# alibaba/nann

Hardware: AMD Instinct MI355X
Metric: retrieval QPS @ recall@200 parity, 1M items/128-d (higher is better)
Workload: dtype f16 rows / f32 L2

## Files before the change

### nann_amd/csrc/nann_hip.hip

```cpp
#include "nann_eval.h"
#include "nann_attn.h"
#include "nann_order_kernels.h"
#include "nann_scan.h"
#include "host/nann_graphdef_text.h"
#include "host/nann_blaze_options.h"
#include "host/nann_npy.h"
#include "host/nann_projcache.h"

#include <algorithm>
#include <atomic>
#include <cmath>
#include <cstddef>
#include <cstdio>
#include <cstdlib>
#include <cstring>
#include <fstream>
#include <limits>
#include <memory>
#include <mutex>
#include <string>
#include <vector>

#include <sys/stat.h>

// ... 548 lines not shown
  const int count = s_count;
  const uint16_t* h = reinterpret_cast<const uint16_t*>(seq_smem);
  for (int k = tid; k < d; k += kSeqMeanThreads) {
    float acc = 0.0f;
    for (int r = 0; r < seq_len; ++r) acc = acc + half_bits_to_float(h[r * d + k]);
    q[(long long)blockIdx.x * d + k] = count ? acc / (float)count : 0.0f;
  }
}

template <int LPR, int DT>
__global__ __launch_bounds__(256) void k_score_l2(const void* table, long long n_table_rows, int d,
                                                  const int32_t* indices, long long n,
                                                  const float* qv, float* scores, OpResult* res) {
  constexpr int GPW = 64 / LPR;
  const int lane = lane_id();
  const int sub = lane % LPR, grp = lane / LPR;
  float q[8];
#pragma unroll
  for (int k = 0; k < 8; ++k) q[k] = qv[sub * 8 + k];
  const long long wave_global = (long long)blockIdx.x * (blockDim.x >> 6) + wave_id();
  const long long n_waves = (long long)gridDim.x * (blockDim.x >> 6);
  for (long long i0 = wave_global * GPW; i0 < n; i0 += n_waves * GPW) {
    const long long i = i0 + grp;
    long long row = -1;
    if (i < n) {
      row = indices ? (long long)indices[i] : i;
      if (row < 0 || row >= n_table_rows) {
        if (sub == 0) atomicMin(reinterpret_cast<unsigned long long*>(&res->bad_i), (unsigned long long)i);
        row = -1;
      }
    }
    float x[8];
    if (row >= 0) {
      const RowChunk<DT> ch = load_chunk<DT>(table, (size_t)row, d, sub);
      chunk_to_float<DT>(ch, x);
    } else {
#pragma unroll
      for (int k = 0; k < 8; ++k) x[k] = 0.0f;
    }
    const float s = l2_finish<LPR>(q, x);
    if (sub == 0 && i < n) scores[i] = s;
  }
}

struct HipProjBackend {
  typedef hipStream_t Stream;
  typedef hipEvent_t Event;
  static bool malloc(void** p, size_t bytes) {
    if (hipMalloc(p, bytes) == hipSuccess) return true;
    (void)hipGetLastError();
    return false;
  }
  static void free(void* p) { (void)hipFree(p); }
  static bool mem_info(size_t* free_b) {
    size_t total = 0;
    if (hipMemGetInfo(free_b, &total) == hipSuccess) return true;
    (void)hipGetLastError();
    return false;
  }
  static bool event_create(Event* e) {
    if (hipEventCreateWithFlags(e, hipEventDisableTiming) == hipSuccess) return true;
    (void)hipGetLastError();
    return false;
  }
  static void event_destroy(Event e) { (void)hipEventDestroy(e); }
  static void event_record(Event e, Stream s) { (void)hipEventRecord(e, s); }
  static bool event_done(Event e) { return hipEventQuery(e) != hipErrorNotReady; }
  static void event_wait(Event e) { (void)hipEventSynchronize(e); }
};
typedef nann::ProjCacheT<HipProjBackend> ProjCache;
typedef nann::ProjTableT<HipProjBackend> ProjTable;
struct SearchOpt {
  int mode;
  int reserve;
  int preproject;
  int mlp_form;
  int small32;
  int order;
};
static std::atomic<int> g_traversal_mode{-1}, g_slot_reserve{-1}, g_preproject{-1};
static const SearchOpt& env_defaults() {
  static const SearchOpt d = [] {
    SearchOpt o{NANN_TRAVERSAL_AUTO, 0, 1, NANN_MLP_FORM_AUTO, 1, 1};
    if (const char* e = std::getenv("NANN_PREPROJECT")) o.preproject = !(e[0] == '0' && e[1] == 0);
    if (const char* e = std::getenv("NANN_SEARCH_SLOT_RESERVE")) o.reserve = std::max(0, std::atoi(e));
    if (const char* e = std::getenv("NANN_MLP_FORM")) o.mlp_form = std::string(e) == "fused" ? NANN_MLP_FORM_FUSED : std::string(e) == "phased" ? NANN_MLP_FORM_PHASED : NANN_MLP_FORM_AUTO;
    if (const char* e = std::getenv("NANN_PHASE_SMALL32")) o.small32 = !(e[0] == '0');
    if (const char* e = std::getenv("NANN_QUERY_ORDER")) o.order = !(e[0] == '0');
    return o;
  }();
  return d;
}
static SearchOpt resolve_options(const nann_search_options* u) {
  SearchOpt o = env_defaults();
  const int gm = g_traversal_mode.load(std::memory_order_relaxed), gr = g_slot_reserve.load(std::memory_order_relaxed),
            gp = g_preproject.load(std::memory_order_relaxed);
  if (gm >= 0) o.mode = gm;
  if (gr >= 0) o.reserve = gr;
  if (gp >= 0) o.preproject = gp;
  if (u) {
    const size_t nb = u->struct_bytes > 0 ? (size_t)u->struct_bytes : sizeof(*u);
    auto has = [&](const int32_t* f) { return (size_t)(reinterpret_cast<const char*>(f) - reinterpret_cast<const char*>(u)) + 4 <= nb; };
    if (has(&u->traversal_mode) && u->traversal_mode >= 0) o.mode = u->traversal_mode;
    if (has(&u->slot_reserve) && u->slot_reserve >= 0) o.reserve = u->slot_reserve;
    if (has(&u->preprojection) && u->preprojection >= 0) o.preproject = u->preprojection != 0;
    if (has(&u->mlp_form) && u->mlp_form >= 0) o.mlp_form = u->mlp_form;
  }
  return o;
}
static int check_options(const nann_search_options* u) {
  if (!u) return NANN_OK;
  if (u->struct_bytes < 0 || (u->struct_bytes > 0 && u->struct_bytes < 8)) return fail(NANN_ERR_BAD_ARGUMENT, "nann_search_options: struct_bytes");
  const SearchOpt o = resolve_options(u);
  if (o.mode < NANN_TRAVERSAL_AUTO || o.mode > NANN_TRAVERSAL_LDS_HASH32) return fail(NANN_ERR_BAD_ARGUMENT, "nann_search_options: unknown traversal_mode");
  if (o.mlp_form < NANN_MLP_FORM_AUTO || o.mlp_form > NANN_MLP_FORM_PHASED) return fail(NANN_ERR_BAD_ARGUMENT, "nann_search_options: unknown mlp_form");
  return NANN_OK;
}

struct nann_scorer {
  nann_scorer_desc desc;
  float* dev_weights = nullptr;
  uint4* dev_packed = nullptr;
  float4* dev_packed_x = nullptr;
  float* dev_cert = nullptr;
  MlpParams mlp = {};
  mutable ProjCache proj;
};

struct nann_attn_scorer {
  AttnParams P = {};
  int emb_dtype = 0;
  int precision = NANN_MLP_EXACT_F32;
  float* dev_weights = nullptr;
  uint4* dev_packed = nullptr;
  mutable ProjCache proj;
};

struct nann_index {
  nann_index_desc desc;
  uint64_t uid = 0;
  bool owns = false;
  std::vector<void*> owned;
  int64_t max_deg[2] = {0, 0};
  uint32_t bm_words = 0;
  bool probe_valid = false;
  int probe_ef = 0, probe_queries = 0;
  float probe_new_per_row_mean = 0.0f, probe_new_per_row_q90 = 0.0f, probe_new_per_row_max = 0.0f;
  float* pivots = nullptr;
  int n_pivots = 0;
};
static void probe_index(nann_index* ix);
static void choose_pivots(nann_index* ix, const std::vector<int32_t>& enter);
static int launch_order(const nann_index* ix, const float* q, int n, int32_t* key, int32_t* perm, unsigned int* heads,
                        hipStream_t st);

extern "C" {

int nann_abi_version(void) { return NANN_ABI_VERSION; }
const char* nann_last_error(void) { return nann::g_err.c_str(); }

int nann_device_count(void) {
  int n = 0;
  if (hipGetDeviceCount(&n) != hipSuccess) return 0;
  return n;
}

int nann_malloc(void** dev_ptr, int64_t nbytes) {
  if (!dev_ptr || nbytes < 0) return fail(NANN_ERR_BAD_ARGUMENT, "nann_malloc: bad argument");
  HIP_TRY(hipMalloc(dev_ptr, (size_t)std::max<int64_t>(nbytes, 1)));
  return NANN_OK;
}

int nann_free(void* dev_ptr) {
  if (dev_ptr) HIP_TRY(hipFree(dev_ptr));
  return NANN_OK;
}

int nann_memcpy(void* dst, const void* src, int64_t nbytes, int kind, nann_stream_t stream) {
  static const hipMemcpyKind kinds[3] = {hipMemcpyHostToDevice, hipMemcpyDeviceToHost,
                                         hipMemcpyDeviceToDevice};
  if (kind < 0 || kind > 2 || nbytes < 0) return fail(NANN_ERR_BAD_ARGUMENT, "nann_memcpy: bad argument");
  if (nbytes == 0) return NANN_OK;
  HIP_TRY(hipMemcpyAsync(dst, src, (size_t)nbytes, kinds[kind], as_stream(stream)));
  return NANN_OK;
}

int nann_stream_synchronize(nann_stream_t stream) {
  HIP_TRY(hipStreamSynchronize(as_stream(stream)));
  return NANN_OK;
}

int nann_stream_create(nann_stream_t* out) {
  if (!out) return fail(NANN_ERR_BAD_ARGUMENT, "nann_stream_create: null argument");
  hipStream_t s = nullptr;
  HIP_TRY(hipStreamCreateWithFlags(&s, hipStreamNonBlocking));
  *out = reinterpret_cast<nann_stream_t>(s);
  return NANN_OK;
}

int nann_stream_destroy(nann_stream_t stream) {
  if (!stream) return NANN_OK;
  HIP_TRY(hipStreamDestroy(as_stream(stream)));
  return NANN_OK;
}

int nann_host_malloc(void** host_ptr, int64_t nbytes) {
  if (!host_ptr || nbytes < 0) return fail(NANN_ERR_BAD_ARGUMENT, "nann_host_malloc: bad argument");
  HIP_TRY(hipHostMalloc(host_ptr, (size_t)std::max<int64_t>(nbytes, 1), hipHostMallocDefault));
  return NANN_OK;
}

int nann_host_free(void* host_ptr) {
  if (!host_ptr) return NANN_OK;
  HIP_TRY(hipHostFree(host_ptr));
  return NANN_OK;
}

static uint16_t f32_to_f16_rne(float f) { return nann_npy::f32_to_f16_rne(f); }

static int read_whole_file(const char* path, std::vector<unsigned char>* out) {
  std::ifstream f(path, std::ifstream::binary | std::ifstream::ate);
  if (!f) return fail(NANN_ERR_IO, std::string("Fail to open file: ") + path);
  const std::streamoff size = f.tellg();
  if (size < 0) return fail(NANN_ERR_IO, std::string("Fail to open file: ") + path);
  out->resize((size_t)size);
  f.seekg(0);
  if (size > 0) f.read(reinterpret_cast<char*>(out->data()), size);
  if (!f || f.gcount() != size) return fail(NANN_ERR_IO, std::string("short read of ") + path);
  return NANN_OK;
}

static int read_npy_host(const char* path, int expect_dtype, const int64_t* expect_shape, int expect_rank,
                         int allow_cast, std::vector<char>* out, std::vector<int64_t>* out_shape) {
  std::vector<unsigned char> image;
  int rc = read_whole_file(path, &image);
  if (rc) return rc;
  const unsigned char* payload = nullptr;
  size_t bytes = 0;
  std::vector<char> conv;
  std::string err;
  rc = nann_npy::decode(image.data(), image.size(), expect_dtype, expect_shape, expect_rank, allow_cast != 0, &payload, &bytes, &conv,
                        out_shape, &err);
  if (rc) return fail(rc, err);
  if (!conv.empty() || bytes == 0) { conv.resize(bytes); out->swap(conv); }
  else out->assign(reinterpret_cast<const char*>(payload), reinterpret_cast<const char*>(payload) + bytes);
  return NANN_OK;
}

int nann_huge_const_load(const char* path, int expect_dtype, const int64_t* expect_shape,
                         int expect_rank, int allow_cast, void** dev_ptr, int64_t* nbytes) {
  if (!path || !dev_ptr) return fail(NANN_ERR_BAD_ARGUMENT, "nann_huge_const_load: null argument");
  std::vector<unsigned char> image;
  int rc = read_whole_file(path, &image);
  if (rc) return rc;
  const unsigned char* payload = nullptr;
  size_t bytes = 0;
  std::vector<char> conv;
  std::string err;
  rc = nann_npy::decode(image.data(), image.size(), expect_dtype, expect_shape, expect_rank, allow_cast != 0, &payload, &bytes, &conv,
                        nullptr, &err);
  if (rc) return fail(rc, err);
  const int64_t total = (int64_t)bytes;
  void* d = nullptr;
  HIP_TRY(hipMalloc(&d, (size_t)std::max<int64_t>(total, 1)));
  if (total) {
    const hipError_t e = hipMemcpy(d, payload, (size_t)total, hipMemcpyHostToDevice);
    if (e != hipSuccess) {
      (void)hipFree(d);
      return fail(NANN_ERR_HIP, std::string("hipMemcpy: ") + hipGetErrorString(e));
    }
  }
  *dev_ptr = d;
  if (nbytes) *nbytes = total;
  return NANN_OK;
}

int nann_group_gather_count(const int64_t* params_row_splits, int64_t n_params_splits,
                            int64_t n_params_values, const int64_t* indices_values,
                            int64_t n_indices_values, const int64_t* indices_row_splits,
                            int64_t n_indices_splits, int64_t* ret_row_splits,
                            int64_t* scratch_offsets, int64_t* n_ret, int64_t* n_ret_splits,
                            int32_t* ragged_code, nann_stream_t stream) {
  if (!n_ret || !n_ret_splits) return fail(NANN_ERR_BAD_ARGUMENT, "nann_group_gather_count: null out");
  ResultBuf* rb;
  int rc = get_result_buf(&rb);
  if (rc) return rc;
  hipStream_t st = as_stream(stream);
  hipLaunchKernelGGL(k_group_gather_count, dim3(1), dim3(kNT), 0, st, params_row_splits,
                     (long long)n_params_splits, (long long)n_params_values, indices_values,
                     (long long)n_indices_values, indices_row_splits, (long long)n_indices_splits,
                     ret_row_splits, scratch_offsets, rb->dev);
  HIP_TRY(hipGetLastError());
  rc = fetch_result(rb, st);
  if (rc) return rc;
  if (ragged_code) *ragged_code = rb->host->code;
  *n_ret = rb->host->n_out;
  *n_ret_splits = rb->host->n_out_splits;
  if (rb->host->err) return fail(rb->host->err, "GroupGather: invalid input, code " +
                                                    std::to_string(rb->host->code));
  return NANN_OK;
}

int nann_group_gather_fill(const int32_t* params_values, const int64_t* params_row_splits,
                           const int64_t* indices_values, int64_t n_indices_values,
                           const int64_t* scratch_offsets, int32_t* ret_values,
                           nann_stream_t stream) {
  if (n_indices_values <= 0) return NANN_OK;
// ... 1115 lines not shown
  o->struct_bytes = (int32_t)sizeof(*o);
  o->traversal_mode = o->slot_reserve = o->preprojection = o->mlp_form = -1;
}

int nann_set_traversal_mode(int32_t mode) {
  if (mode < NANN_TRAVERSAL_AUTO || mode > NANN_TRAVERSAL_LDS_HASH32)
    return fail(NANN_ERR_BAD_ARGUMENT, "nann_set_traversal_mode: unknown mode");
  g_traversal_mode.store(mode, std::memory_order_relaxed);
  return NANN_OK;
}

int nann_search_workspace_bytes(const nann_index* ix, const int32_t level_topn[6], int64_t n_queries,
                                int64_t* nbytes) {
  if (!ix || !level_topn || !nbytes) return fail(NANN_ERR_BAD_ARGUMENT, "nann_search_workspace_bytes: null argument");
  SearchPlan p;
  const int rc = plan_search(ix, level_topn, n_queries, -1, &p, resolve_options(nullptr));
  if (rc) return rc;
  *nbytes = (int64_t)(256 + p.slot_bytes * (unsigned long long)std::max(p.slots, p.fb_slots) + kPhaseTail +
                      order_ws_bytes(n_queries));
  return NANN_OK;
}

}


template <typename Build>
static int projection_for(ProjCache& c, const nann_index* ix, int width, hipStream_t st, Build build, bool pin, bool enabled,
                          std::shared_ptr<ProjTable>* out) {
  const size_t bytes = (size_t)ix->desc.n_items * (size_t)width * 4;
  return c.acquire(ix->uid, bytes, enabled, pin, [&](float* t) -> int {
    const int rc = build(t);
    if (rc) return rc;
    const hipError_t e = hipStreamSynchronize(st);
    if (e != hipSuccess) return fail(NANN_ERR_HIP, std::string("pre-projection: ") + hipGetErrorString(e));
    return NANN_OK;
  }, out);
}

static void projection_used(ProjCache& c, const std::shared_ptr<ProjTable>& tab, hipStream_t st) { c.used(tab, st); }

static int projection_release(ProjCache& c, const nann_index* ix) {
  if (c.release(ix->uid)) return NANN_OK;
  return fail(NANN_ERR_BAD_ARGUMENT, "release: no pre-projected table of this index");
}

static int mlp_projection(const nann_scorer* sc, const nann_index* ix, hipStream_t st, bool pin, bool enabled, std::shared_ptr<ProjTable>* out) {
  return projection_for(sc->proj, ix, kMlpProjWidth, st, [&](float* t) {
    return launch_mlp_preproject(ix->desc.emb_dtype, ix->desc.item_embs, (long long)ix->desc.n_items, ix->desc.d, sc->mlp.w1, t, st);
  }, pin, enabled, out);
}

static int attn_projection(const nann_attn_scorer* sc, const nann_index* ix, hipStream_t st, bool pin, bool enabled, std::shared_ptr<ProjTable>* out) {
  return projection_for(sc->proj, ix, kAttnProjWidth, st, [&](float* t) {
    return launch_attn_preproject(ix->desc.emb_dtype, sc->P, ix->desc.item_embs, (long long)ix->desc.n_items, t, st);
  }, pin, enabled, out);
}

static int launch_search_any(int lpr, int dt, int kind, int split, int vis, int nt, int slots, size_t lds_bytes,
                             const SearchArgs& a, hipStream_t st) {
  if (kind == NANN_SCORER_MLP) {
    if (lpr == 8) return launch_search_mlp_d64(dt, split, vis, slots, lds_bytes, a, st);
    if (lpr == 16) return launch_search_mlp_d128(dt, split, vis, slots, lds_bytes, a, st);
    if (lpr == 32) return launch_search_mlp_d256(dt, split, vis, slots, lds_bytes, a, st);
    return fail(NANN_ERR_UNSUPPORTED, "MLP scorer: d <= 256 only");
  }
  if (dt == NANN_F16) return launch_search_l2_f16(lpr, vis, nt, slots, lds_bytes, a, st);
  if (dt == NANN_BF16) return launch_search_l2_bf16(lpr, vis, nt, slots, lds_bytes, a, st);
  return launch_search_l2_f32(lpr, vis, nt, slots, lds_bytes, a, st);
}

extern "C" {

int nann_search(const nann_index* ix, const nann_scorer* scorer, const float* q, int64_t n_queries,
                const int32_t level_topn[6], void* workspace, int64_t workspace_bytes,
                int64_t* out_item_ids, float* out_scores, int32_t* out_index, int32_t* status,
                int32_t* counters, nann_stream_t stream) {
  return nann_search_opt(ix, scorer, q, n_queries, level_topn, nullptr, workspace, workspace_bytes, out_item_ids, out_scores,
                         out_index, status, counters, nullptr, nullptr, nullptr, stream);
}

}

static int search_impl(const nann_index* ix, const nann_scorer* scorer, const nann_attn_scorer* attn,
                       const float* q, const float* kt, const float* upad, int64_t n_queries,
                       const int32_t level_topn[6], const int32_t* tq, void* workspace, int64_t workspace_bytes,
                       int64_t* out_item_ids, float* out_scores, int32_t* out_index, int32_t* status,
                       int32_t* counters, int64_t* phase_ticks, const nann_search_options* options, nann_search_plan* plan_out,
                       hipStream_t st) {
  if (n_queries > 0x7fffffffll) return fail(NANN_ERR_UNSUPPORTED, "too many queries in one call");
  int rc = check_options(options);
  if (rc) return rc;
  SearchOpt opt = resolve_options(options);
  const int kind = attn ? kKindAttn : scorer->desc.kind;
  const bool mlp = !attn && kind == NANN_SCORER_MLP;
  const bool mlp_split = mlp && scorer->desc.precision == NANN_MLP_SPLIT_F16;
  const bool mlp_cert = mlp && scorer->desc.precision == NANN_MLP_CERTIFIED;
  if (mlp_cert && opt.mlp_form == NANN_MLP_FORM_FUSED) opt.mlp_form = NANN_MLP_FORM_PHASED;
  std::shared_ptr<ProjTable> tab;
  ProjCache* cache = nullptr;
  if (attn) {
    cache = &attn->proj;
    rc = attn_projection(attn, ix, st, false, opt.preproject != 0, &tab);
  } else if (mlp) {
    cache = &scorer->proj;
    rc = mlp_projection(scorer, ix, st, false, opt.preproject != 0, &tab);
  }
  if (rc) return rc;
  const bool mlp_res = mlp && tab;
  SearchPlan p;
  rc = plan_search(ix, level_topn, n_queries, mlp_res ? kKindMlpRes : mlp_split ? kKindMlpSplit : kind, &p, opt, mlp && !mlp_split);
  if (rc) return rc;
  if (plan_out) {
    const bool ph = mlp_res && p.phased;
    const int v = ph ? p.phase_vis : p.vis;
    plan_out->visited_set = v == VIS_LDS_HASH ? NANN_TRAVERSAL_LDS_HASH : v == VIS_LDS_HASH32 ? NANN_TRAVERSAL_LDS_HASH32
                            : v == VIS_LDS_BITMAP ? NANN_TRAVERSAL_LDS_BITMAP : NANN_TRAVERSAL_HBM_BITMAP;
    plan_out->fallback_visited_set = p.fb_vis == VIS_LDS_BITMAP ? NANN_TRAVERSAL_LDS_BITMAP : NANN_TRAVERSAL_HBM_BITMAP;
    plan_out->threads = ph ? (p.phase_vis == VIS_LDS_HASH32 ? kNT : 512) : ((mlp || attn) && p.nt == kNT ? 512 : p.nt);
    plan_out->workgroups = ph ? p.phase_slots : p.slots;
    plan_out->phased = ph ? 1 : 0;
    plan_out->table = tab ? 1 : 0;
    plan_out->est_visited = p.est_visited;
    plan_out->worst_visited = p.worst_visited;
  }
  const int64_t need_slots = p.phased ? std::max<int64_t>(std::min<int64_t>(n_queries, kPhaseChunk), p.fb_slots) : std::max(p.slots, p.fb_slots);
  if (!workspace || workspace_bytes < (int64_t)(256 + p.slot_bytes * (unsigned long long)need_slots + (p.phased ? kPhaseTail : 0)))
    return fail(NANN_ERR_CAPACITY, "workspace smaller than nann_search_workspace_bytes()");
  SearchArgs a;
  a.emb = ix->desc.item_embs;
  a.item_ids = ix->desc.item_ids;
  for (int l = 0; l < 2; ++l) { a.nbv[l] = ix->desc.nb_values[l]; a.nbrs[l] = ix->desc.nb_row_splits[l]; }
  a.enter = ix->desc.enter_points;
  a.n_enter = (int)ix->desc.n_enter;
  a.n_items = (uint32_t)ix->desc.n_items;
  a.d = ix->desc.d;
  a.q = q;
  a.n_queries = (int)n_queries;
  for (int i = 0; i < 6; ++i) a.t[i] = level_topn[i];
  a.tq = tq;
  a.ws = static_cast<unsigned char*>(workspace);
  a.slot_bytes = p.slot_bytes;
  a.bm_words = ix->bm_words;
  a.max_cand = p.max_cand; a.max_raw = p.max_raw; a.pool_cap = p.pool_cap;
  a.out_ids = out_item_ids; a.out_scores = out_scores; a.out_index = out_index;
  a.status = status; a.counters = counters;
  a.phase_ticks = reinterpret_cast<long long*>(phase_ticks);
  a.id_bits = p.id_bits;
  a.redo = 0;
  a.phase = 0;
  a.proj = tab ? tab->table : nullptr;
  a.mlp = MlpParams{};
  a.attn = AttnParams{};
  a.kt = kt; a.upad = upad;
  HIP_TRY(hipMemsetAsync(workspace, 0, 256, st));
  const int dt = ix->desc.emb_dtype;
  const bool hashed = p.vis == VIS_LDS_HASH || p.vis == VIS_LDS_HASH32;
  const unsigned long long slots_end = 256 + p.slot_bytes * (unsigned long long)std::max(p.slots, p.fb_slots) + kPhaseTail;
  const unsigned long long order_off = ((unsigned long long)workspace_bytes - order_ws_bytes(n_queries)) & ~255ull;
  if (opt.order && hashed && !attn && kind == NANN_SCORER_L2 && ix->n_pivots >= 2 && n_queries > p.slots &&
      (unsigned long long)workspace_bytes >= ((slots_end + 255) & ~255ull) + order_ws_bytes(n_queries)) {
    unsigned char* ow = static_cast<unsigned char*>(workspace) + order_off;
    unsigned int* heads = reinterpret_cast<unsigned int*>(ow);
    int32_t* perm = reinterpret_cast<int32_t*>(ow + kOrderSegs * kOrderHeadStride * 4);
    int32_t* key = perm + n_queries;
    rc = launch_order(ix, q, (int)n_queries, key, perm, heads, st);
    if (rc) return rc;
    a.perm = perm;
    a.xheads = heads;
  }
  auto both = [&](auto&& launch_on) -> int {
    int r2 = launch_on(p.vis, p.nt, p.slots, p.lds_bytes);
    if (!r2 && hashed) {
      a.redo = 1;
      a.perm = nullptr;
      a.xheads = nullptr;
      r2 = launch_on(p.fb_vis, kNT, p.fb_slots, p.fb_lds_bytes);
    }
    if (cache) projection_used(*cache, tab, st);
    return r2;
  };
  if (attn) {
    a.attn = attn->P;
    if (tab) {
      auto launch = attn->precision == NANN_MLP_SPLIT_F16 ? launch_search_attn_proj : launch_search_attn_xproj;
      const bool resident = attn->precision == NANN_MLP_SPLIT_F16;
      return both([&](int vis, int, int slots, size_t lds) {
        if (resident && vis == VIS_LDS_HASH && !a.redo) return launch_search_attn_res(slots, lds, a, st);
        return launch(vis, slots, lds, a, st);
      });
    }
    auto launch = attn->precision == NANN_MLP_SPLIT_F16 ? launch_search_attn_split : launch_search_attn;
    return both([&](int vis, int, int slots, size_t lds) { return launch(ix->desc.d, dt, vis, slots, lds, a, st); });
  }
  a.mlp = scorer->mlp;
  a.phase = 0;
  const int exact = scorer->desc.kind == NANN_SCORER_MLP && (scorer->desc.precision == NANN_MLP_EXACT_F32 || mlp_cert);
  if (mlp_res && p.phased) {
    DeviceInfo di;
    rc = device_info(&di);
    if (rc) return rc;
    const int k5 = level_topn[5];
    for (int64_t c0 = 0; c0 < n_queries && !rc; c0 += kPhaseChunk) {
      SearchArgs c = a;
      c.n_queries = (int)std::min<int64_t>(kPhaseChunk, n_queries - c0);
      c.q = q + (size_t)c0 * a.d;
      if (tq) c.tq = tq + (size_t)c0 * 6;
      c.out_ids = out_item_ids + (size_t)c0 * k5;
      if (out_scores) c.out_scores = out_scores + (size_t)c0 * k5;
      if (out_index) c.out_index = out_index + (size_t)c0 * k5;
      c.status = status + c0;
      if (counters) c.counters = counters + (size_t)c0 * 3 * NANN_NUM_ROUNDS;
      if (phase_ticks) c.phase_ticks = reinterpret_cast<long long*>(phase_ticks) + (size_t)c0 * NANN_NUM_PHASES;
      if (c0 && mlp_cert) {
        HIP_TRY(hipMemsetAsync(workspace, 0, offsetof(WsHeader, refined), st));
        HIP_TRY(hipMemsetAsync(static_cast<unsigned char*>(workspace) + offsetof(WsHeader, pad2), 0, 256 - offsetof(WsHeader, pad2), st));
      } else if (c0) HIP_TRY(hipMemsetAsync(workspace, 0, 256, st));
      const int slots = (int)std::min<int64_t>(c.n_queries, (int64_t)p.phase_slots);
      for (int ph = 0; ph <= NANN_NUM_ROUNDS && !rc; ++ph) {
        c.phase = ph;
        rc = launch_search_mlp_phase(p.phase_vis, slots, p.phase_lds_bytes, c, st);
        if (!rc && ph < NANN_NUM_ROUNDS) {
          rc = mlp_cert ? launch_mlp_phase_certified(c, ph, p.phase_score_wgs, st)
                        : launch_mlp_phase_score(exact, c, ph, p.phase_score_wgs, st);
        }
      }
      if (!rc) {
        c.redo = 1;
        c.phase = 0;
        rc = launch_search_mlp_res(exact, p.fb_vis, p.fb_slots, p.fb_lds_bytes, c, st);
      }
    }
    if (cache) projection_used(*cache, tab, st);
    return rc;
  }
  if (mlp_res)
    return both([&](int vis, int, int slots, size_t lds) {
      return launch_search_mlp_res(exact, vis, slots, lds, a, st);
    });
  return both([&](int vis, int nt, int slots, size_t lds) {
    return launch_search_any(ix->desc.d / 8, dt, kind, mlp_split, vis, nt, slots, lds, a, st);
  });
}

__global__ void k_probe_queries(const void* emb, int dt, int d, long long n_items, int nq, float* q) {
  const int j = blockIdx.x;
  const long long row = (long long)j * (n_items / nq);
  for (int k = threadIdx.x; k < d; k += blockDim.x) {
    float v;
    if (dt == NANN_F32) v = static_cast<const float*>(emb)[row * d + k];
    else {
      const uint32_t h = static_cast<const uint16_t*>(emb)[row * d + k];
      v = dt == NANN_F16 ? half_bits_to_float(h) : bf16_bits_to_float(h);
    }
    q[(size_t)j * d + k] = v;
  }
}

__global__ void k_order_gather(const void* emb, int dt, int d, const int32_t* rows, int m, float* out) {
  for (int k = threadIdx.x; k < d; k += blockDim.x) out[(size_t)blockIdx.x * d + k] = order_row_elem(emb, dt, (size_t)rows[blockIdx.x] * d + k);
}

static int launch_order(const nann_index* ix, const float* q, int n, int32_t* key, int32_t* perm, unsigned int* heads,
                        hipStream_t st) {
  const int d = ix->desc.d, P = ix->n_pivots;
  const size_t lds = ((size_t)d * P + kOrderMaxPivots + (size_t)kOrderKeyQueries * d) * 4;
  if (lds > 48 * 1024)
    HIP_TRY(hipFuncSetAttribute(reinterpret_cast<const void*>(k_order_key), hipFuncAttributeMaxDynamicSharedMemorySize, (int)lds));
  hipLaunchKernelGGL(k_order_key, dim3((unsigned)((n + kOrderKeyQueries - 1) / kOrderKeyQueries)), dim3(256), lds, st,
                     ix->pivots, d, P, q, n, key);
  HIP_TRY(hipGetLastError());
  hipLaunchKernelGGL(k_order_perm, dim3(1), dim3(kOrderSortThreads), 0, st, key, n, P, perm, heads);
  HIP_TRY(hipGetLastError());
  return NANN_OK;
}

static void choose_pivots(nann_index* ix, const std::vector<int32_t>& enter) {
  const int d = ix->desc.d;
  const int P = order_pivots((int64_t)enter.size(), d);
  if (P < 2) return;
  constexpr size_t kMaxCand = 1024;
  const size_t E = enter.size(), m = std::min(E, kMaxCand);
  std::vector<int32_t> cand(m);
  for (size_t i = 0; i < m; ++i) cand[i] = enter[i * E / m];
  int32_t* rows = nullptr;
  float* buf = nullptr;
  std::vector<float> x(m * (size_t)d);
  bool ok = hipMalloc(&rows, m * 4) == hipSuccess && hipMalloc(&buf, m * (size_t)d * 4) == hipSuccess &&
            hipMemcpy(rows, cand.data(), m * 4, hipMemcpyHostToDevice) == hipSuccess;
  if (ok) {
    hipLaunchKernelGGL(k_order_gather, dim3((unsigned)m), dim3(128), 0, nullptr, ix->desc.item_embs, ix->desc.emb_dtype, d, rows, (int)m, buf);
    ok = hipGetLastError() == hipSuccess && hipMemcpy(x.data(), buf, x.size() * 4, hipMemcpyDeviceToHost) == hipSuccess;
  }
  if (buf) (void)hipFree(buf);
  if (rows) (void)hipFree(rows);
  if (!ok) return;
  std::vector<size_t> piv;
  std::vector<double> dist(m, INFINITY);
  size_t cur = 0;
  for (int p = 0; p < P; ++p) {
    piv.push_back(cur);
    size_t far = cur;
    for (size_t i = 0; i < m; ++i) {
      double s = 0.0;
      for (int k = 0; k < d; ++k) { const double t = (double)x[i * d + k] - (double)x[cur * d + k]; s += t * t; }
      dist[i] = std::min(dist[i], s);
      if (dist[i] > dist[far]) far = i;
    }
    if (dist[far] <= 0.0) break;
    cur = far;
  }
  if (piv.size() < 2) return;
  const size_t np = piv.size();
  std::vector<float> t((size_t)d * np + kOrderMaxPivots, 0.0f);
  for (size_t p = 0; p < np; ++p) {
    float s = 0.0f;
    for (int k = 0; k < d; ++k) {
      const float v = x[piv[p] * d + k];
      t[(size_t)k * np + p] = v;
      s += v * v;
    }
    t[(size_t)d * np + p] = s;
  }
  float* dev = nullptr;
  if (hipMalloc(&dev, t.size() * 4) != hipSuccess) return;
  if (hipMemcpy(dev, t.data(), t.size() * 4, hipMemcpyHostToDevice) != hipSuccess) { (void)hipFree(dev); return; }
  ix->pivots = dev;
  ix->n_pivots = (int)piv.size();
}

static void probe_index(nann_index* ix) {
  ix->probe_valid = false;
  static const bool enabled = [] { const char* e = std::getenv("NANN_INDEX_PROBE"); return !(e && e[0] == '0'); }();
  if (!enabled) return;
  const std::string saved_error = nann::g_err;
  struct RestoreError { const std::string& s; ~RestoreError() { nann::g_err = s; } } restore{saved_error};
  const int d = ix->desc.d;
  const int64_t E = ix->desc.n_enter, N = ix->desc.n_items;
  if (E < 8 || N < 4096) return;
  const int nq = 64, e = (int)std::min<int64_t>(64, E);
  const int32_t t[6] = {e, e, e, e, e, std::min(e, 10)};
  nann_scorer_desc sd{};
  sd.kind = NANN_SCORER_L2; sd.d = d; sd.emb_dtype = ix->desc.emb_dtype;
  nann_scorer* sc = nullptr;
  if (nann_scorer_create(&sd, &sc) != NANN_OK) return;
  nann_search_options o;
  nann_search_options_init(&o);
  o.traversal_mode = NANN_TRAVERSAL_HBM_BITMAP;
  o.slot_reserve = 0;
  int64_t ws_bytes = 0;
  const size_t n_ctr = (size_t)nq * 3 * NANN_NUM_ROUNDS;
  unsigned char* buf = nullptr;
  std::vector<int32_t> h_ctr(n_ctr), h_st((size_t)nq);
  bool ok = nann_search_workspace_bytes(ix, t, nq, &ws_bytes) == NANN_OK;
  const size_t off_q = ((size_t)ws_bytes + 255) & ~(size_t)255, off_ids = off_q + (size_t)nq * d * 4,
               off_st = off_ids + (size_t)nq * t[5] * 8, off_ctr = off_st + (size_t)nq * 4, total = off_ctr + n_ctr * 4;
  ok = ok && hipMalloc(reinterpret_cast<void**>(&buf), total) == hipSuccess;
  if (ok) {
    hipStream_t st = nullptr;
    hipLaunchKernelGGL(k_probe_queries, dim3(nq), dim3(128), 0, st, ix->desc.item_embs, ix->desc.emb_dtype, d, (long long)N, nq,
                       reinterpret_cast<float*>(buf + off_q));
    ok = search_impl(ix, sc, nullptr, reinterpret_cast<const float*>(buf + off_q), nullptr, nullptr, nq, t, nullptr, buf, ws_bytes,
                     reinterpret_cast<int64_t*>(buf + off_ids), nullptr, nullptr, reinterpret_cast<int32_t*>(buf + off_st),
                     reinterpret_cast<int32_t*>(buf + off_ctr), nullptr, &o, nullptr, st) == NANN_OK;
    ok = ok && hipMemcpy(h_ctr.data(), buf + off_ctr, n_ctr * 4, hipMemcpyDeviceToHost) == hipSuccess &&
         hipMemcpy(h_st.data(), buf + off_st, (size_t)nq * 4, hipMemcpyDeviceToHost) == hipSuccess;
  }
  if (buf) (void)hipFree(buf);
  nann_scorer_destroy(sc);
  if (!ok) (void)hipGetLastError();
  if (!ok) return;
  double sum = 0.0, mx = 0.0;
  int n_valid = 0;
  std::vector<double> ratios;
  for (int j = 0; j < nq; ++j) {
    if (h_st[(size_t)j] != NANN_OK) continue;
    const int32_t* c = h_ctr.data() + (size_t)j * 3 * NANN_NUM_ROUNDS;
    double rows = 0.0, fresh = 0.0;
    for (int r = 2; r <= 4; ++r) { rows += c[0 * NANN_NUM_ROUNDS + r]; fresh += c[2 * NANN_NUM_ROUNDS + r]; }
    if (rows <= 0.0) continue;
    const double ratio = fresh / rows;
    sum += ratio; mx = std::max(mx, ratio);
    ratios.push_back(ratio);
    ++n_valid;
  }
  if (n_valid < 8) return;
  ix->probe_valid = true;
  ix->probe_ef = e;
  ix->probe_queries = n_valid;
  std::sort(ratios.begin(), ratios.end());
  ix->probe_new_per_row_mean = (float)(sum / n_valid);
  ix->probe_new_per_row_q90 = (float)ratios[(size_t)(0.9 * (double)(n_valid - 1))];
  ix->probe_new_per_row_max = (float)mx;
}

extern "C" {

int nann_search_ex(const nann_index* ix, const nann_scorer* scorer, const float* q, int64_t n_queries,
                   const int32_t level_topn[6], void* workspace, int64_t workspace_bytes,
                   int64_t* out_item_ids, float* out_scores, int32_t* out_index, int32_t* status,
                   int32_t* counters, int64_t* phase_ticks, nann_stream_t stream) {
  return nann_search_opt(ix, scorer, q, n_queries, level_topn, nullptr, workspace, workspace_bytes, out_item_ids, out_scores,
                         out_index, status, counters, phase_ticks, nullptr, nullptr, stream);
}

int nann_search_opt(const nann_index* ix, const nann_scorer* scorer, const float* q, int64_t n_queries,
                    const int32_t level_topn_max[6], const int32_t* level_topn, void* workspace, int64_t workspace_bytes,
                    int64_t* out_item_ids, float* out_scores, int32_t* out_index, int32_t* status, int32_t* counters,
                    int64_t* phase_ticks, const nann_search_options* options, nann_search_plan* plan, nann_stream_t stream) {
  if (!ix || !scorer || !level_topn_max || !out_item_ids || !status)
    return fail(NANN_ERR_BAD_ARGUMENT, "nann_search_opt: null argument");
  if (n_queries <= 0) return NANN_OK;
  if (scorer->desc.d != ix->desc.d || scorer->desc.emb_dtype != ix->desc.emb_dtype)
    return fail(NANN_ERR_BAD_ARGUMENT, "scorer and index disagree on d / dtype");
  if (level_topn && phase_ticks) return fail(NANN_ERR_UNSUPPORTED, "nann_search_opt: phase ticks with a uniform level_topn only");
  return search_impl(ix, scorer, nullptr, q, nullptr, nullptr, n_queries, level_topn_max, level_topn, workspace, workspace_bytes,
                     out_item_ids, out_scores, out_index, status, counters, phase_ticks, options, plan, as_stream(stream));
}

int nann_search_reruns(const void* workspace, int64_t* n_rerun, nann_stream_t stream) {
  if (!workspace || !n_rerun) return fail(NANN_ERR_BAD_ARGUMENT, "nann_search_reruns: null argument");
  unsigned int v = 0;
  HIP_TRY(hipMemcpyAsync(&v, static_cast<const unsigned char*>(workspace) + offsetof(WsHeader, n_redo), 4, hipMemcpyDeviceToHost, as_stream(stream)));
  HIP_TRY(hipStreamSynchronize(as_stream(stream)));
  *n_rerun = v;
// ... 519 lines not shown
```

### nann_amd/csrc/nann_order.h

```cpp
#pragma once
#include <hip/hip_runtime.h>
#include <hip/hip_fp16.h>
#include <stdint.h>
#include <algorithm>
#include <cmath>
#include "../../include/nann_hip.h"

namespace nann {

constexpr int kOrderSegs = 8;
constexpr int kOrderHeadStride = 32;
constexpr int kOrderMaxPivots = 128;
constexpr int kOrderPivotLds = 64 * 1024;
constexpr int kOrderKeyQueries = 16;
constexpr int kOrderSortThreads = 1024;

__host__ __device__ inline int order_seg_begin(int n, int s) { return (int)((long long)n * s / kOrderSegs); }

inline int order_pivots(int64_t n_enter, int d) {
  return (int)std::min<int64_t>(n_enter, std::min(kOrderMaxPivots, kOrderPivotLds / (4 * d)));
}

inline unsigned long long order_ws_bytes(int64_t n) {
  return ((unsigned long long)kOrderSegs * kOrderHeadStride * 4 + (unsigned long long)n * 8 + 255) / 256 * 256;
}

__device__ inline unsigned int xcc_id() {
#if defined(__HIP_DEVICE_COMPILE__)
  unsigned int x;
  asm volatile("s_getreg_b32 %0, hwreg(HW_REG_XCC_ID, 0, 4)" : "=s"(x));
  return x;
#else
  return 0;
#endif
}

}
```

### nann_amd/csrc/nann_order_kernels.h

```cpp
#pragma once
#include "nann_order.h"

namespace nann {

__device__ inline float order_row_elem(const void* emb, int dt, size_t i) {
  if (dt == NANN_F32) return reinterpret_cast<const float*>(emb)[i];
  const uint16_t h = reinterpret_cast<const uint16_t*>(emb)[i];
  if (dt == NANN_F16) return __half2float(__ushort_as_half(h));
  return __uint_as_float((uint32_t)h << 16);
}

__global__ __launch_bounds__(256) void k_order_key(const float* pivT, int d, int P, const float* q, int n, int32_t* key) {
  extern __shared__ float4 order_lds4[];
  float* piv = reinterpret_cast<float*>(order_lds4);
  float* qs = piv + (size_t)d * P + kOrderMaxPivots;
  const int q0 = blockIdx.x * kOrderKeyQueries, nq = min(kOrderKeyQueries, n - q0);
  const int pv4 = (d * P + kOrderMaxPivots) / 4, qv4 = nq * d / 4;
  for (int i = threadIdx.x; i < pv4; i += 256) order_lds4[i] = reinterpret_cast<const float4*>(pivT)[i];
  for (int i = threadIdx.x; i < qv4; i += 256)
    reinterpret_cast<float4*>(qs)[i] = reinterpret_cast<const float4*>(q + (size_t)q0 * d)[i];
  __syncthreads();
  const int lane = threadIdx.x & 63, wave = threadIdx.x >> 6;
  const int pa = lane, pb = lane + 64;
  float acc[4][2] = {};
  const float* qw = qs + (size_t)wave * 4 * d;
  for (int k = 0; k < d; ++k) {
    const float va = piv[k * P + min(pa, P - 1)], vb = piv[k * P + min(pb, P - 1)];
#pragma unroll
    for (int j = 0; j < 4; ++j) {
      const float x = qw[j * d + k];
      acc[j][0] = fmaf(x, va, acc[j][0]);
      acc[j][1] = fmaf(x, vb, acc[j][1]);
    }
  }
  const float* pn = piv + (size_t)d * P;
#pragma unroll
  for (int j = 0; j < 4; ++j) {
    const int qi = wave * 4 + j;
    float best = pa < P ? fmaf(-2.0f, acc[j][0], pn[min(pa, P - 1)]) : INFINITY;
    int arg = pa < P ? pa : 0x7fffffff;
    if (pb < P) {
      const float s = fmaf(-2.0f, acc[j][1], pn[pb]);
      if (s < best) { best = s; arg = pb; }
    }
    for (int m = 32; m >= 1; m >>= 1) {
      const float ob = __shfl_xor(best, m);
      const int oa = __shfl_xor(arg, m);
      if (ob < best || (ob == best && oa < arg)) { best = ob; arg = oa; }
    }
    if (lane == 0 && qi < nq) key[q0 + qi] = arg < P ? arg : 0;
  }
}

__global__ __launch_bounds__(kOrderSortThreads) void k_order_perm(const int32_t* key, int n, int P, int32_t* perm,
                                                                 unsigned int* heads) {
  constexpr int W = kOrderSortThreads / 64;
  __shared__ int base[kOrderMaxPivots];
  __shared__ int wofs[W][kOrderMaxPivots];
  const int tid = threadIdx.x, lane = tid & 63, w = tid >> 6;
  if (tid < kOrderSegs * kOrderHeadStride) heads[tid] = 0u;
  for (int p = tid; p < P; p += blockDim.x) base[p] = 0;
  __syncthreads();
  for (int i = tid; i < n; i += blockDim.x) atomicAdd(&base[key[i]], 1);
  __syncthreads();
  int pre = 0;
  if (tid < P)
    for (int p = 0; p < tid; ++p) pre += base[p];
  __syncthreads();
  if (tid < P) base[tid] = pre;
  __syncthreads();
  for (int t0 = 0; t0 < n; t0 += kOrderSortThreads) {
    for (int i = tid; i < W * kOrderMaxPivots; i += blockDim.x) (&wofs[0][0])[i] = 0;
    __syncthreads();
    const int i = t0 + tid;
    const int k = i < n ? key[i] : -1;
    int rank = 0;
    bool last = true;
#pragma unroll
    for (int j = 0; j < 64; ++j) {
      const int kj = __builtin_amdgcn_readlane(k, j);
      if (kj == k) { if (j < lane) ++rank; else if (j > lane) last = false; }
    }
    if (k >= 0 && last) wofs[w][k] = rank + 1;
    __syncthreads();
    for (int p = tid; p < P; p += blockDim.x) {
      int run = base[p];
      for (int v = 0; v < W; ++v) { const int c = wofs[v][p]; wofs[v][p] = run; run += c; }
      base[p] = run;
    }
    __syncthreads();
    if (k >= 0) perm[wofs[w][k] + rank] = i;
    __syncthreads();
  }
}

}
```

Baseline: 2.790 million.

## Speed up query-order permutation with ballot-based ranking and single-pass scan

Rewrites k_order_perm to rank equal keys within a wave using seven ballots and mbcnt instead of a 64-step readlane loop. For up to 8192 queries it adds a fast path that builds per-run u16 counts in LDS and does one block-wide prefix scan, cutting the tiled passes and barriers. The fallback path's serial prefix sum becomes a wave scan. The kernel also clears the workspace header, which removes a separate hipMemsetAsync on the ordered path. This adds assumptions about key width (seven bits) and u16 counts.

```diff
diff --git a/nann_amd/csrc/nann_hip.hip b/nann_amd/csrc/nann_hip.hip
--- a/nann_amd/csrc/nann_hip.hip
+++ b/nann_amd/csrc/nann_hip.hip
@@ -724,7 +724,7 @@
 static void probe_index(nann_index* ix);
 static void choose_pivots(nann_index* ix, const std::vector<int32_t>& enter);
 static int launch_order(const nann_index* ix, const float* q, int n, int32_t* key, int32_t* perm, unsigned int* heads,
-                        hipStream_t st);
+                        unsigned int* header, hipStream_t st);
 
 extern "C" {
 
@@ -2146,7 +2146,6 @@
   a.mlp = MlpParams{};
   a.attn = AttnParams{};
   a.kt = kt; a.upad = upad;
-  HIP_TRY(hipMemsetAsync(workspace, 0, 256, st));
   const int dt = ix->desc.emb_dtype;
   const bool hashed = p.vis == VIS_LDS_HASH || p.vis == VIS_LDS_HASH32;
   const unsigned long long slots_end = 256 + p.slot_bytes * (unsigned long long)std::max(p.slots, p.fb_slots) + kPhaseTail;
@@ -2157,10 +2156,12 @@
     unsigned int* heads = reinterpret_cast<unsigned int*>(ow);
     int32_t* perm = reinterpret_cast<int32_t*>(ow + kOrderSegs * kOrderHeadStride * 4);
     int32_t* key = perm + n_queries;
-    rc = launch_order(ix, q, (int)n_queries, key, perm, heads, st);
+    rc = launch_order(ix, q, (int)n_queries, key, perm, heads, static_cast<unsigned int*>(workspace), st);
     if (rc) return rc;
     a.perm = perm;
     a.xheads = heads;
+  } else {
+    HIP_TRY(hipMemsetAsync(workspace, 0, 256, st));
   }
   auto both = [&](auto&& launch_on) -> int {
     int r2 = launch_on(p.vis, p.nt, p.slots, p.lds_bytes);
@@ -2254,8 +2255,9 @@
   for (int k = threadIdx.x; k < d; k += blockDim.x) out[(size_t)blockIdx.x * d + k] = order_row_elem(emb, dt, (size_t)rows[blockIdx.x] * d + k);
 }
 
+static_assert(sizeof(WsHeader) <= kOrderHeaderWords * 4 && kOrderHeaderWords * 4 == 256, "k_order_perm clears the header");
 static int launch_order(const nann_index* ix, const float* q, int n, int32_t* key, int32_t* perm, unsigned int* heads,
-                        hipStream_t st) {
+                        unsigned int* header, hipStream_t st) {
   const int d = ix->desc.d, P = ix->n_pivots;
   const size_t lds = ((size_t)d * P + kOrderMaxPivots + (size_t)kOrderKeyQueries * d) * 4;
   if (lds > 48 * 1024)
@@ -2263,7 +2265,7 @@
   hipLaunchKernelGGL(k_order_key, dim3((unsigned)((n + kOrderKeyQueries - 1) / kOrderKeyQueries)), dim3(256), lds, st,
                      ix->pivots, d, P, q, n, key);
   HIP_TRY(hipGetLastError());
-  hipLaunchKernelGGL(k_order_perm, dim3(1), dim3(kOrderSortThreads), 0, st, key, n, P, perm, heads);
+  hipLaunchKernelGGL(k_order_perm, dim3(1), dim3(kOrderSortThreads), 0, st, key, n, P, perm, heads, header);
   HIP_TRY(hipGetLastError());
   return NANN_OK;
 }
diff --git a/nann_amd/csrc/nann_order.h b/nann_amd/csrc/nann_order.h
--- a/nann_amd/csrc/nann_order.h
+++ b/nann_amd/csrc/nann_order.h
@@ -13,7 +13,14 @@
 constexpr int kOrderMaxPivots = 128;
 constexpr int kOrderPivotLds = 64 * 1024;
 constexpr int kOrderKeyQueries = 16;
+static_assert(kOrderKeyQueries % 4 == 0, "a key workgroup is 4 waves");
 constexpr int kOrderSortThreads = 1024;
+constexpr int kOrderFastQueries = 8192;
+constexpr int kOrderFastRuns = kOrderFastQueries / 64;
+static_assert(kOrderFastQueries % kOrderSortThreads == 0 && kOrderFastQueries < 65536, "u16 prefixes, whole tiles");
+static_assert(kOrderMaxPivots * kOrderFastRuns == 16 * kOrderSortThreads, "the scan gives each thread 16 table entries");
+static_assert(kOrderMaxPivots == 128, "a key is seven bits (order_same_key)");
+constexpr int kOrderHeaderWords = 64;
 
 __host__ __device__ inline int order_seg_begin(int n, int s) { return (int)((long long)n * s / kOrderSegs); }
 
diff --git a/nann_amd/csrc/nann_order_kernels.h b/nann_amd/csrc/nann_order_kernels.h
--- a/nann_amd/csrc/nann_order_kernels.h
+++ b/nann_amd/csrc/nann_order_kernels.h
@@ -22,12 +22,13 @@
   __syncthreads();
   const int lane = threadIdx.x & 63, wave = threadIdx.x >> 6;
   const int pa = lane, pb = lane + 64;
-  float acc[4][2] = {};
-  const float* qw = qs + (size_t)wave * 4 * d;
+  constexpr int QW = kOrderKeyQueries / 4;
+  float acc[QW][2] = {};
+  const float* qw = qs + (size_t)wave * QW * d;
   for (int k = 0; k < d; ++k) {
     const float va = piv[k * P + min(pa, P - 1)], vb = piv[k * P + min(pb, P - 1)];
 #pragma unroll
-    for (int j = 0; j < 4; ++j) {
+    for (int j = 0; j < QW; ++j) {
       const float x = qw[j * d + k];
       acc[j][0] = fmaf(x, va, acc[j][0]);
       acc[j][1] = fmaf(x, vb, acc[j][1]);
@@ -35,8 +36,8 @@
   }
   const float* pn = piv + (size_t)d * P;
 #pragma unroll
-  for (int j = 0; j < 4; ++j) {
-    const int qi = wave * 4 + j;
+  for (int j = 0; j < QW; ++j) {
+    const int qi = wave * QW + j;
     float best = pa < P ? fmaf(-2.0f, acc[j][0], pn[min(pa, P - 1)]) : INFINITY;
     int arg = pa < P ? pa : 0x7fffffff;
     if (pb < P) {
@@ -52,36 +53,105 @@
   }
 }
 
+__device__ inline unsigned long long order_same_key(int k) {
+  unsigned long long m = __ballot(k >= 0);
+#pragma unroll
+  for (int b = 0; b < 7; ++b) {
+    const unsigned long long s = __ballot((k >> b) & 1);
+    m &= ((k >> b) & 1) ? s : ~s;
+  }
+  return m;
+}
+
+__device__ inline int order_rank(unsigned long long m) {
+  return (int)__builtin_amdgcn_mbcnt_hi((unsigned int)(m >> 32), __builtin_amdgcn_mbcnt_lo((unsigned int)m, 0u));
+}
+
+__device__ inline int order_wave_scan(int v, int lane) {
+#pragma unroll
+  for (int s = 1; s < 64; s <<= 1) {
+    const int o = __shfl_up(v, s);
+    if (lane >= s) v += o;
+  }
+  return v;
+}
+
 __global__ __launch_bounds__(kOrderSortThreads) void k_order_perm(const int32_t* key, int n, int P, int32_t* perm,
-                                                                 unsigned int* heads) {
+                                                                 unsigned int* heads, unsigned int* header) {
   constexpr int W = kOrderSortThreads / 64;
+  __shared__ __attribute__((aligned(16))) uint16_t cnt[kOrderMaxPivots * kOrderFastRuns];
+  __shared__ int wtot[W];
   __shared__ int base[kOrderMaxPivots];
   __shared__ int wofs[W][kOrderMaxPivots];
-  const int tid = threadIdx.x, lane = tid & 63, w = tid >> 6;
+  const int tid = threadIdx.x, lane = tid & 63, w = __builtin_amdgcn_readfirstlane(tid >> 6);
   if (tid < kOrderSegs * kOrderHeadStride) heads[tid] = 0u;
-  for (int p = tid; p < P; p += blockDim.x) base[p] = 0;
+  if (tid < kOrderHeaderWords) header[tid] = 0u;
+  if (n <= kOrderFastQueries) {
+    constexpr int T = kOrderFastQueries / kOrderSortThreads;
+    int k[T], rank[T];
+#pragma unroll
+    for (int t = 0; t < T; ++t) {
+      const int i = t * kOrderSortThreads + tid;
+      k[t] = i < n ? key[i] : -1;
+    }
+    uint4* cnt4 = reinterpret_cast<uint4*>(cnt);
+    cnt4[tid] = make_uint4(0u, 0u, 0u, 0u);
+    cnt4[tid + kOrderSortThreads] = make_uint4(0u, 0u, 0u, 0u);
+    __syncthreads();
+#pragma unroll
+    for (int t = 0; t < T; ++t) {
+      rank[t] = 0;
+      if ((t * W + w) * 64 < n) {
+        const unsigned long long m = order_same_key(k[t]);
+        rank[t] = order_rank(m);
+        if (k[t] >= 0 && (m >> lane) == 1ull) cnt[k[t] * kOrderFastRuns + t * W + w] = (uint16_t)(rank[t] + 1);
+      }
+    }
+    __syncthreads();
+    const uint4 lo = cnt4[2 * tid], hi = cnt4[2 * tid + 1];
+    const uint32_t v[8] = {lo.x, lo.y, lo.z, lo.w, hi.x, hi.y, hi.z, hi.w};
+    int sum = 0;
+#pragma unroll
+    for (int j = 0; j < 8; ++j) sum += (int)(v[j] & 0xffffu) + (int)(v[j] >> 16);
+    const int incl = order_wave_scan(sum, lane);
+    if (lane == 63) wtot[w] = incl;
+    __syncthreads();
+    uint32_t run = (uint32_t)(incl - sum);
+    for (int x = 0; x < w; ++x) run += (uint32_t)wtot[x];
+    uint32_t o[8];
+#pragma unroll
+    for (int j = 0; j < 8; ++j) {
+      const uint32_t c0 = v[j] & 0xffffu, c1 = v[j] >> 16;
+      o[j] = run | ((run + c0) << 16);
+      run += c0 + c1;
+    }
+    cnt4[2 * tid] = make_uint4(o[0], o[1], o[2], o[3]);
+    cnt4[2 * tid + 1] = make_uint4(o[4], o[5], o[6], o[7]);
+    __syncthreads();
+#pragma unroll
+    for (int t = 0; t < T; ++t)
+      if (k[t] >= 0) perm[(int)cnt[k[t] * kOrderFastRuns + t * W + w] + rank[t]] = t * kOrderSortThreads + tid;
+    return;
+  }
+  for (int p = tid; p < kOrderMaxPivots; p += blockDim.x) base[p] = 0;
   __syncthreads();
   for (int i = tid; i < n; i += blockDim.x) atomicAdd(&base[key[i]], 1);
   __syncthreads();
-  int pre = 0;
-  if (tid < P)
-    for (int p = 0; p < tid; ++p) pre += base[p];
-  __syncthreads();
-  if (tid < P) base[tid] = pre;
+  if (w == 0) {
+    const int c0 = base[2 * lane], c1 = base[2 * lane + 1];
+    const int pre = order_wave_scan(c0 + c1, lane) - (c0 + c1);
+    base[2 * lane] = pre;
+    base[2 * lane + 1] = pre + c0;
+  }
   __syncthreads();
   for (int t0 = 0; t0 < n; t0 += kOrderSortThreads) {
     for (int i = tid; i < W * kOrderMaxPivots; i += blockDim.x) (&wofs[0][0])[i] = 0;
     __syncthreads();
     const int i = t0 + tid;
     const int k = i < n ? key[i] : -1;
-    int rank = 0;
-    bool last = true;
-#pragma unroll
-    for (int j = 0; j < 64; ++j) {
-      const int kj = __builtin_amdgcn_readlane(k, j);
-      if (kj == k) { if (j < lane) ++rank; else if (j > lane) last = false; }
-    }
-    if (k >= 0 && last) wofs[w][k] = rank + 1;
+    const unsigned long long m = order_same_key(k);
+    const int rank = order_rank(m);
+    if (k >= 0 && (m >> lane) == 1ull) wofs[w][k] = rank + 1;
     __syncthreads();
     for (int p = tid; p < P; p += blockDim.x) {
       int run = base[p];
```

Result: faster. 2.853 million, median of 6 (+2.3%).
